# srihari-humbarwadi/retinanet-tensorflow2.x

Measured on AMD Instinct MI355X. Metric: images/sec train, ResNet50-640 RetinaNet data-parallel step (encode + fwd + loss + bwd + clip + all-reduce + SGD/EMA); inference images/s under `infer`, higher is better.
Workload: dtype bf16; 1 GPU; ResNet50-640x640 bf16 training, 32 images/GPU (BASELINE configs[2] shard: global batch 32), resnet_initial frozen, single GPU; global_batch=32, parallelism=dp1, rccl_ranks=1, comm=torch, syncbn_messages=0

## Files before the change

### include/rnet_hip.h

```cpp
#ifndef RNET_HIP_H_
#define RNET_HIP_H_

#include <stddef.h>
#include <stdint.h>

#ifdef __cplusplus
extern "C" {
#endif
#if defined(__GNUC__)
#pragma GCC visibility push(default)
#endif

typedef enum {
  RN_OK = 0,
  RN_EINVAL = -1,
  RN_ENOMEM = -2,
  RN_EHIP = -3,
  RN_ECOMM = -4,
  RN_EUNSUPPORTED = -5
} rn_status;

enum { RN_DT_F32 = 0, RN_DT_BF16 = 1 };
enum { RN_ACT_NONE = 0, RN_ACT_RELU = 1, RN_ACT_RELU6 = 2, RN_ACT_SWISH = 3 };

// ... 84 lines not shown

typedef struct {
  const void* x;
  const void* w;
  void* y;
  const float* scale;
  const float* shift;
  const void* residual;
  int32_t N, H, W, Cin, pix_stride, Ho, Wo, Cout;
  float* bn_partial;
  const float* bias;
  int32_t w_terms;
  int32_t w_pair;
  const void* bn_bwd_y;
  const float* bn_bwd_fwd;
} rn_conv_segment;

typedef struct {
  int32_t R, S, stride_h, stride_w, pad_top, pad_left;
  int32_t act;
  int32_t out_dtype;
  int32_t num_segments;
  rn_conv_segment seg[RN_CONV_MAX_SEGMENTS];
  rn_launch_opts opts;
  void* splitk_ws;
  int64_t splitk_ws_bytes;
} rn_conv_problem;

int rn_conv2d_nhwc_fwd(const rn_conv_problem* problem , void* stream);
size_t rn_conv_splitk_workspace_bytes(const rn_conv_problem* problem );
size_t rn_conv_splitk_workspace_max_bytes(void);

int rn_conv_cout_pad(int Cout);
int rn_conv_tile_rows(const rn_conv_problem* problem);
int rn_conv_bn_row_blocks(const rn_conv_problem* problem, int segment);
int rn_conv_kernel_id(const rn_conv_problem* problem);
int rn_conv_cin_pad(int Cin);
int rn_pack_conv_weight(const float* w_hwio, int R, int S, int Cin, int Cout, int Cin_pad, void* w_packed,
                        void* stream);
int rn_pack_conv_weight_split(const float* w, int layout_ohwi, int R, int S, int Cin, int Cout, int Cin_pad, int terms,
                              void* w_packed, void* stream);
int rn_conv_pair_rows(int Cout);
int rn_pack_conv_weight_pair(const float* w, int layout_ohwi, int R, int S, int Cin, int Cout, int Cin_pad,
                             void* w_packed, void* stream);
int rn_pack_conv_weight_ohwi(const float* w_ohwi, int R, int S, int Cin, int Cout, int Cin_pad, void* w_packed,
                             void* stream);
int rn_pack_stem_weight(const float* w_hwio, int Cout, void* w_packed, void* stream);
int rn_stem_padded_width(int W);
int rn_pack_stem_input(const float* images, int N, int H, int W, void* packed, void* stream);
int rn_pack_stem_weight_rs(const float* w_hwio, int R, int S, int Cout, void* w_packed, void* stream);
int rn_pack_image_nhwc4(const float* images, int N, int H, int W, int pad_top, int pad_left, int Hp, int Wp,
// ... 226 lines not shown
```

### retinanet-tensorflow2.x_amd/csrc/rn_conv.hip

```cpp
#include <map>
#include <mutex>
#include <tuple>

#include <algorithm>
#include "rn_conv_dev.h"

template <int BM, int BN, int BK, bool OUT_F32, int ABL = 0, int WM = 2, int WN = 2, int STAGES = 2, bool SPLIT = false>
__global__ void __launch_bounds__(64 * WM * WN, 2) conv_fwd_kernel(const ConvArgs args) {
  constexpr int NWAVES = WM * WN;
  constexpr int NTHREADS = 64 * NWAVES;
  constexpr int SLOTS = BK / 8;
  constexpr int RPI = 64 / SLOTS;
  constexpr int A_INSTR = BM / RPI / NWAVES;
  constexpr int B_INSTR = BN / RPI / NWAVES;
  constexpr int WTM = BM / WM, WTN = BN / WN;
  constexpr int TM = WTM / 32, TN = WTN / 32;
  constexpr int KSUB = BK / 16;
  constexpr int A_BYTES = BM * BK * 2, B_BYTES = BN * BK * 2;
  constexpr int STAGE_BYTES = A_BYTES + B_BYTES;
  static_assert(A_INSTR >= 1 && B_INSTR >= 1, "tile too small for the wave count");

  extern __shared__ __attribute__((aligned(16))) char smem[];

  int tile, part = 0;
// ... 401 lines not shown
        }
#pragma unroll
        for (int q = 0; q < 4; ++q) {
          float t = f4[q] + sbs[q];
          if (round1) t = rn_rb(t);
          if (affine) t = t * ssc[q] + ssf[q];
          if (round2) t = rn_rb(t);
          f4[q] = t;
        }
        v = make_float4(f4[0], f4[1], f4[2], f4[3]);
      } else {
        v = *(const float4*)(cl + rr * BN + ec);
      }
      const long long o = (long long)m * Cout + n;
      if (sg.residual) {
        const uint2 rv = *(const uint2*)(sg.residual + o);
        v.x += rn_bf16_to_f32((uint16_t)(rv.x & 0xffffu));
        v.y += rn_bf16_to_f32((uint16_t)(rv.x >> 16));
        v.z += rn_bf16_to_f32((uint16_t)(rv.y & 0xffffu));
        v.w += rn_bf16_to_f32((uint16_t)(rv.y >> 16));
      }
      {
        float f4[4] = {v.x, v.y, v.z, v.w};
        if (!OUT_F32 && args.act == RN_ACT_SWISH) {
#pragma unroll
          for (int q = 0; q < 4; ++q) f4[q] = rn_rb(f4[q]);
        }
        rn_apply_act_n<4>(f4, args.act);
        v = make_float4(f4[0], f4[1], f4[2], f4[3]);
      }
      if ((ABL & 8) && v.x != 123.456f) continue;
// ... 278 lines not shown
  const int mc = conv_splitk_min_chunks(p);
  if (!mc) return 0;
  long long tiles = 0;
  for (int i = 0; i < p->num_segments; ++i) {
    const rn_conv_segment& s = p->seg[i];
    tiles += rn_cdiv((long long)s.N * s.Ho * s.Wo, 256) * rn_cdiv(rn_conv_cout_pad(seg_cols(s)), 256);
  }
  long long bytes = 0;
  splitk_parts((int)tiles, mc, rn_persistent_grid(0x7fffffff, rn_num_cus(), p->opts), &bytes);
  return (size_t)bytes;
}

extern "C" int rn_conv_kernel_id(const rn_conv_problem* p) {
  if (!p || p->num_segments < 1 || p->num_segments > RN_CONV_MAX_SEGMENTS) return -1;
  return conv_pick(p);
}

extern "C" int rn_conv_bn_row_blocks(const rn_conv_problem* p, int segment) {
  if (!p || p->num_segments < 1 || p->num_segments > RN_CONV_MAX_SEGMENTS || segment < 0 || segment >= p->num_segments) return 0;
  const int kid = conv_pick(p);
  const long long M = (long long)p->seg[segment].N * p->seg[segment].Ho * p->seg[segment].Wo;
  if (kid == 1) {
    const int r = conv_big_balanced_rows(p);
    if (r) return (int)(2 * rn_cdiv(M, r));
  }
  const int rows = kid == 3 ? 512 : (kid ? 256 : 128);
  return (int)((rows / 128) * rn_cdiv(M, rows));
}

extern "C" int rn_conv_tile_rows(const rn_conv_problem* p) {
// ... 59 lines not shown
    RN_CHECK_ARG(s.Cout % 4 == 0, "rn_conv2d_nhwc_fwd: segment %d Cout=%d not a multiple of 4", i, s.Cout);
    const int cp = rn_conv_cout_pad(seg_cols(s));
    RN_CHECK_ARG((cp <= 64) == (cout_pad0 <= 64), "rn_conv2d_nhwc_fwd: segments mix Cout tile widths");
    RN_CHECK_ARG(!s.w_pair || ((big || halo512) && p->out_dtype == RN_DT_F32 && s.w_terms <= 1 && !s.scale && !s.shift &&
                               !s.residual && !s.bn_partial),
                 "rn_conv2d_nhwc_fwd: segment %d: w_pair needs an f32 launch without scale / shift / residual that the 256- / "
                 "512-row kernels take (rn_conv_kernel_id() != 0)", i);
    RN_CHECK_ARG(((uintptr_t)s.x | (uintptr_t)s.w | (uintptr_t)s.y | (uintptr_t)s.residual) % 16 == 0,
                 "rn_conv2d_nhwc_fwd: segment %d tensors must be 16-byte aligned", i);
    const long long M = (long long)s.N * s.Ho * s.Wo;
    RN_CHECK_ARG(M < (1ll << 31) && (long long)s.N * s.H * s.W * s.pix_stride * 2 < (1ll << 31),
                 "rn_conv2d_nhwc_fwd: segment %d input exceeds the 2 GiB buffer-addressing limit", i);
    ConvSegDev& d = a.seg[ii];
    d.x = (const uint16_t*)s.x; d.w = (const uint16_t*)s.w; d.y = s.y;
    d.scale = s.scale; d.shift = s.shift; d.residual = (const uint16_t*)s.residual;
    d.bn_partial = s.bn_partial;
    d.bn_y = (const uint16_t*)s.bn_bwd_y;
    d.bn_fwd = s.bn_bwd_fwd;
    if (s.bn_bwd_y) {
      RN_CHECK_ARG(s.bn_partial && s.bn_bwd_fwd && p->out_dtype == RN_DT_BF16 && !s.scale && !s.shift && !s.bias &&
                       !s.residual && p->act == RN_ACT_NONE && s.Cout % 8 == 0 && (uintptr_t)s.bn_bwd_y % 16 == 0,
                   "rn_conv2d_nhwc_fwd: segment %d: bn_bwd_y needs bn_partial + bn_bwd_fwd on a plain bf16 launch", i);
    }
    RN_CHECK_ARG((s.bn_bwd_y != nullptr) == (p->seg[0].bn_bwd_y != nullptr),
                 "rn_conv2d_nhwc_fwd: bn_bwd_y must be set on all segments or none");
    d.bias = s.bias;
    d.N = s.N; d.H = s.H; d.W = s.W; d.Cin = s.Cin; d.pix_stride = s.pix_stride;
    d.Ho = s.Ho; d.Wo = s.Wo; d.Cout = seg_cols(s);
    d.pair_cout = s.w_pair ? s.Cout : 0;
    d.rows = kid == 1 ? bal_rows : 0;
// ... 239 lines not shown
```

### retinanet-tensorflow2.x_amd/csrc/rn_conv_big.hip

```cpp
#include "rn_conv_big_epi.h"

namespace {

constexpr int BM = 256, BN = 256, BK = 32, NW = 8, STAGES = 4;
constexpr int A_BYTES = BM * BK * 2, STAGE_BYTES = (BM + BN) * BK * 2;
constexpr int RING_BYTES = STAGES * STAGE_BYTES, PATCH_BYTES = 4096;
constexpr int LDS_BYTES = RING_BYTES + NW * PATCH_BYTES;

template <bool OUT_F32, bool HAS_RES, bool BN_BWD = false>
__global__ void __launch_bounds__(512) conv_big_kernel(const ConvArgs args) {
  extern __shared__ __attribute__((aligned(16))) char smem[];
  const int total = args.total_tiles;
  const int G = gridDim.x;
  const int tid = threadIdx.x;
  const int lane = tid & 63;
  const int wave = __builtin_amdgcn_readfirstlane(tid >> 6);
  const int wave_m = wave >> 2, wave_n = wave & 3;
  const int R = args.R, S = args.S, RS = R * S;

  int i_v = blockIdx.x;
  int i_tap = 0, i_c0 = 0;
  int i_r = 0, i_s = 0;
  int g_iss = 0;
  int i_W = 0, i_PS = 0, i_Cin = 0, i_cw = 0;
  __amdgpu_buffer_rsrc_t rs_x, rs_w;
// ... 145 lines not shown
    _Pragma("unroll 1") for (int i = 1; i < args.nseg; ++i)                                           \
      if (tile__ >= args.seg[i].tile_begin) c_si = i;                                                 \
    const ConvSegDev& sg__ = args.seg[c_si];                                                          \
    const int lt__ = tile__ - sg__.tile_begin;                                                        \
    const int mt__ = rn_fdiv(lt__, sg__.n_tiles, rn_rcp((float)sg__.n_tiles));   \
    const int rows_t__ = sg__.rows ? sg__.rows : BM;                                                  \
    c_m0 = mt__ * rows_t__;                                                                           \
    c_mend = c_m0 + rows_t__ < sg__.M ? c_m0 + rows_t__ : sg__.M;                                     \
    c_chunk0 = mt__ * 2;                                                                              \
    c_n0 = (lt__ - mt__ * sg__.n_tiles) * BN;                                                         \
    c_ksteps = RS * (sg__.CinP / BK);                                                                 \
    c_k = 0;                                                                                          \
  } while (0)

  auto epilogue = [&]() __attribute__((always_inline)) {
    big_epilogue<OUT_F32, HAS_RES, BN_BWD>(acc, args, c_si, c_m0, c_n0, wave, smem + RING_BYTES + wave * PATCH_BYTES,
                                           BigEpiSrc(), c_mend, c_chunk0);
  };

  BIG_SETUP_ISSUE();
  BIG_SETUP_COMPUTE();
  big_acc_init<OUT_F32, HAS_RES>(acc, args, c_si, c_n0, wave);
#pragma unroll 1
  for (int t = 0; t < 3 && i_v < total; ++t) BIG_ISSUE_STEP();
  if (g_iss >= 3) asm volatile("s_waitcnt vmcnt(4)" ::: "memory");
  else asm volatile("s_waitcnt vmcnt(0)" ::: "memory");
  BIG_BARRIER();
  BIG_LOADSEG(0);
  if (wave_m == 1) BIG_BARRIER();

#define BIG_TILE_END()                                       \
// ... 14 lines not shown
    if (wave_m == 1) BIG_BARRIER();
    ++g;
    BIG_LOADSEG(g & 3);
    BIG_BARRIER();
  }
#undef BIG_TILE_END
#undef BIG_SETUP_COMPUTE
#undef BIG_BARRIER
#undef BIG_COMPUTESEG
#undef BIG_LOADSEG
#undef BIG_READ
#undef BIG_ISSUE_STEP
#undef BIG_SETUP_ISSUE
}

}

int rn_launch_conv_big(const ConvArgs& a, bool out_f32, const rn_launch_opts& opts, hipStream_t st) {
  static unsigned long long attr_set = 0;
  if (RN_ATTRS_NEEDED(attr_set)) {
    RN_CHECK_HIP(hipFuncSetAttribute((const void*)conv_big_kernel<false, false>,
                                     hipFuncAttributeMaxDynamicSharedMemorySize, LDS_BYTES));
    RN_CHECK_HIP(hipFuncSetAttribute((const void*)conv_big_kernel<false, true>,
                                     hipFuncAttributeMaxDynamicSharedMemorySize, LDS_BYTES));
    RN_CHECK_HIP(hipFuncSetAttribute((const void*)conv_big_kernel<true, false>,
                                     hipFuncAttributeMaxDynamicSharedMemorySize, LDS_BYTES));
    RN_CHECK_HIP(hipFuncSetAttribute((const void*)conv_big_kernel<true, true>,
                                     hipFuncAttributeMaxDynamicSharedMemorySize, LDS_BYTES));
    RN_CHECK_HIP(hipFuncSetAttribute((const void*)conv_big_kernel<false, false, true>,
                                     hipFuncAttributeMaxDynamicSharedMemorySize, LDS_BYTES));
    RN_ATTRS_DONE(attr_set);
  }
  const int grid = rn_persistent_grid(a.total_tiles, rn_num_cus(), opts);
  bool has_res = false;
  for (int i = 0; i < a.nseg; ++i) has_res = has_res || a.seg[i].residual != nullptr;
  const dim3 g3(grid), b3(512);
  if (a.seg[0].bn_y) {
    hipLaunchKernelGGL((conv_big_kernel<false, false, true>), g3, b3, LDS_BYTES, st, a);
  } else if (out_f32) {
    if (has_res) hipLaunchKernelGGL((conv_big_kernel<true, true>), g3, b3, LDS_BYTES, st, a);
    else hipLaunchKernelGGL((conv_big_kernel<true, false>), g3, b3, LDS_BYTES, st, a);
  } else {
    if (has_res) hipLaunchKernelGGL((conv_big_kernel<false, true>), g3, b3, LDS_BYTES, st, a);
    else hipLaunchKernelGGL((conv_big_kernel<false, false>), g3, b3, LDS_BYTES, st, a);
  }
  RN_CHECK_LAUNCH();
  return RN_OK;
}
```

### retinanet-tensorflow2.x_amd/csrc/rn_conv_big_epi.h

```cpp
#ifndef RN_CONV_BIG_EPI_H_
#define RN_CONV_BIG_EPI_H_
#include <type_traits>

#include "rn_conv_dev.h"

#ifdef HALO_PROF
__device__ unsigned long long g_halo_clk[48];
#define EPI_STAMP(k_) if (blockIdx.x == 0 && threadIdx.x == 0) g_halo_clk[k_] = clock64();
#else
#define EPI_STAMP(k_)
#endif

#ifdef HALO_ABLATE
#define EPI_ABLATE HALO_ABLATE
#else
#define EPI_ABLATE 0
#endif

typedef rn_h16 bf16x2_t __attribute__((ext_vector_type(2)));
typedef float f32x2_t __attribute__((ext_vector_type(2)));

__device__ __forceinline__ uint32_t pack2(float lo, float hi) {
  f32x2_t v = {lo, hi};
  bf16x2_t b = __builtin_convertvector(v, bf16x2_t);
// ... 96 lines not shown
#pragma unroll
  for (int j = 0; j < NJ; ++j)
#pragma unroll
    for (int q = 0; q < 4; ++q) {
      float a0 = __uint_as_float(v[0][j][q].x), a1 = __uint_as_float(v[0][j][q].y);
      float a2 = __uint_as_float(v[0][j][q].z), a3 = __uint_as_float(v[0][j][q].w);
#pragma unroll
      for (int p = 1; p < 4; ++p) {
        a0 += __uint_as_float(v[p][j][q].x); a1 += __uint_as_float(v[p][j][q].y);
        a2 += __uint_as_float(v[p][j][q].z); a3 += __uint_as_float(v[p][j][q].w);
      }
      t[j][q * 4] = a0; t[j][q * 4 + 1] = a1; t[j][q * 4 + 2] = a2; t[j][q * 4 + 3] = a3;
    }
}

template <bool OUT_F32, bool HAS_RES, bool BN_BWD = false, bool FROM_WS = false, int WM = 2>
__device__ __forceinline__ void big_epilogue(f32x16_t (&acc)[4][2], const ConvArgs& args, int c_si, int c_m0,
                                             int c_n0, int wave, char* patch, const BigEpiSrc src = BigEpiSrc(),
                                             int m_end = -1, int chunk0 = -1) {
  static_assert(!(BN_BWD && (OUT_F32 || HAS_RES)), "BN_BWD: plain bf16 launches only");
  constexpr bool LOADS = HAS_RES || BN_BWD;
  const int wave_m = wave / (8 / WM), wave_n = wave % (8 / WM);
  const ConvSegDev& sg = args.seg[c_si];
  const int Cout = sg.Cout, M = m_end >= 0 ? m_end : sg.M;
  const int nw0 = c_n0 + wave_n * 64;
  const int mw0 = c_m0 + wave_m * 128;
  const int elane = (int)__builtin_amdgcn_mbcnt_hi(~0u, __builtin_amdgcn_mbcnt_lo(~0u, 0u));
  const int fr = elane & 31, fh = elane >> 5;
  const int rrow = elane >> 3, ru = elane & 7;
  if (!OUT_F32) {
    const int nr = nw0 + ru * 8;
    const bool nok = nr < Cout;
    float sc[8], sf[8];
#pragma unroll
    for (int q = 0; q < 8; ++q) { sc[q] = 1.0f; sf[q] = 0.0f; }
// ... 33 lines not shown
    EPI_STAMP(12);
    const bool has_res = HAS_RES && sg.residual != nullptr;
    const uint16_t* const side = BN_BWD ? sg.bn_y : sg.residual;
    const bool has_side = BN_BWD ? true : has_res;
    const bool stats = sg.bn_partial != nullptr;
    float st0[8], st1[8];
#pragma unroll
    for (int q = 0; q < 8; ++q) st0[q] = st1[q] = 0.0f;
    char* const ybase = (char*)sg.y + ((long long)(mw0 + rrow) * Cout + nr) * 2;
    const long long row_bytes = (long long)Cout * 2;
    const int act = args.act;
    const bool clamp_lo = act == RN_ACT_RELU || act == RN_ACT_RELU6, clamp_hi = act == RN_ACT_RELU6;
    const bool affine = !BN_BWD && (sg.scale != nullptr || sg.shift != nullptr);
    const bool plain = BN_BWD || (!affine && !has_res && act != RN_ACT_SWISH);
    const bool round2 = affine && has_res;
    uint4 rv[2][LOADS ? 4 : 1];
#define BIG_RES_PREFETCH(buf_, i_)                                                                    \
_Pragma("unroll") for (int pass = 0; pass < (LOADS ? 4 : 0); ++pass) {                              \
  const int m = mw0 + (i_) * 32 + pass * 8 + rrow;                                                  \
  rv[buf_][pass] = make_uint4(0u, 0u, 0u, 0u);                                                      \
  if (has_side && nok && m < M) rv[buf_][pass] = *(const uint4*)(side + (long long)m * Cout + nr);  \
}
    const uint32_t lo2 = clamp_lo ? 0u : 0x80008000u, hi2 = clamp_hi ? RN_SIX_X2 : 0x7fff7fffu;
    auto blocks = [&](auto plain_c, auto stats_c, auto round2_c, auto swish_c) __attribute__((always_inline)) {
      constexpr bool PLAIN = decltype(plain_c)::value;
      constexpr int STATS = decltype(stats_c)::value, ROUND2 = decltype(round2_c)::value, SWISH = decltype(swish_c)::value;
      BIG_RES_PREFETCH(0, 0);
#pragma unroll
      for (int i = 0; i < 4; ++i) {
        EPI_STAMP(13 + 2 * i);
        if (i + 1 < 4) BIG_RES_PREFETCH((i + 1) & 1, i + 1);
        if (FROM_WS) big_epi_rebuild<2>(&acc[i][0], src, i, 0);
#pragma unroll
        for (int j = 0; j < 2; ++j)
#pragma unroll
          for (int g = 0; g < 4; ++g) {
            const int nl = j * 32 + g * 8 + fh * 4;
            uint2 pk;
            pk.x = pack2(acc[i][j][g * 4 + 0], acc[i][j][g * 4 + 1]);
            pk.y = pack2(acc[i][j][g * 4 + 2], acc[i][j][g * 4 + 3]);
            *(uint2*)(patch + fr * 128 + (((nl >> 3) ^ (fr & 7)) << 4) + ((((nl >> 2) ^ (fr >> 3)) & 1) << 3)) = pk;
          }
        EPI_STAMP(14 + 2 * i);
        uint4 vb[4];
#pragma unroll
        for (int pass = 0; pass < 4; ++pass) {
          const int row = pass * 8 + rrow;
          const uint4 t = *(const uint4*)(patch + row * 128 + ((ru ^ (row & 7)) << 4));
          vb[pass] = (pass & 1) ? make_uint4(t.z, t.w, t.x, t.y) : t;
        }
#pragma unroll
        for (int pass = 0; pass < 4; ++pass) {
          const int row = pass * 8 + rrow;
          const uint4 v = vb[pass];
          const int m = mw0 + i * 32 + row;
          if (m < M && nok) {
            uint4 ov;
            if (PLAIN) {
              ov.x = pk_min_i16(pk_max_i16(v.x, lo2), hi2); ov.y = pk_min_i16(pk_max_i16(v.y, lo2), hi2);
              ov.z = pk_min_i16(pk_max_i16(v.z, lo2), hi2); ov.w = pk_min_i16(pk_max_i16(v.w, lo2), hi2);
            } else {
              const uint4 r4 = HAS_RES ? rv[i & 1][LOADS ? pass : 0] : make_uint4(0u, 0u, 0u, 0u);
              float f[8] = {bf_lo(v.x), bf_hi(v.x), bf_lo(v.y), bf_hi(v.y), bf_lo(v.z), bf_hi(v.z), bf_lo(v.w), bf_hi(v.w)};
              const float rr[8] = {bf_lo(r4.x), bf_hi(r4.x), bf_lo(r4.y), bf_hi(r4.y),
                                   bf_lo(r4.z), bf_hi(r4.z), bf_lo(r4.w), bf_hi(r4.w)};
#pragma unroll
              for (int q = 0; q < 8; ++q) f[q] = f[q] * sc[q] + sf[q];
              if (ROUND2 == 1 || (ROUND2 == 2 && round2)) {
#pragma unroll
                for (int q = 0; q < 8; q += 2) {
                  const uint32_t pq = pack2(f[q], f[q + 1]);
                  f[q] = bf_lo(pq); f[q + 1] = bf_hi(pq);
                }
              }
#pragma unroll
              for (int q = 0; q < 8; ++q) f[q] += rr[q];
              if (SWISH == 1 || (SWISH == 2 && act == RN_ACT_SWISH)) {
#pragma unroll
                for (int q = 0; q < 8; ++q) f[q] = rn_swish(rn_rb(f[q]));
              }
              ov.x = pack2(f[0], f[1]); ov.y = pack2(f[2], f[3]); ov.z = pack2(f[4], f[5]); ov.w = pack2(f[6], f[7]);
              ov.x = pk_min_i16(pk_max_i16(ov.x, lo2), hi2); ov.y = pk_min_i16(pk_max_i16(ov.y, lo2), hi2);
// ... 13 lines not shown
                  st0[q] += g;
                  st1[q] += g * ((yy[q] - mu[BN_BWD ? q : 0]) * is[BN_BWD ? q : 0]);
                }
              } else {
#pragma unroll
                for (int q = 0; q < 8; ++q) { st0[q] += w[q]; st1[q] += w[q] * w[q]; }
              }
            }
          }
        }
      }
    };
    typedef std::integral_constant<int, 0> off_t;
    typedef std::integral_constant<int, 1> on_t;
    typedef std::integral_constant<int, 2> runtime_t;
    if constexpr (BN_BWD) {
      blocks(std::true_type{}, on_t{}, off_t{}, off_t{});
    } else if (plain) {
      if (stats) blocks(std::true_type{}, on_t{}, off_t{}, off_t{});
      else blocks(std::true_type{}, off_t{}, off_t{}, off_t{});
    } else if (!stats && act != RN_ACT_SWISH) {
      if (round2) blocks(std::false_type{}, off_t{}, on_t{}, off_t{});
      else blocks(std::false_type{}, off_t{}, off_t{}, off_t{});
    } else {
      blocks(std::false_type{}, runtime_t{}, runtime_t{}, runtime_t{});
    }
    EPI_STAMP(21);
    if (stats) {
#pragma unroll
      for (int q = 0; q < 8; ++q) {
#pragma unroll
// ... 67 lines not shown
```

### retinanet-tensorflow2.x_amd/csrc/rn_conv_dev.h

```cpp
#ifndef RN_CONV_DEV_H_
#define RN_CONV_DEV_H_
#include "rn_common.h"

typedef rn_h16 bf16x8_t __attribute__((ext_vector_type(8)));
typedef float f32x16_t __attribute__((ext_vector_type(16)));

#define CONV_THREADS 256

struct ConvSegDev {
  const uint16_t* x;
  const uint16_t* w;
  void* y;
  const float* scale;
  const float* shift;
  const uint16_t* residual;
  float* bn_partial;
  const float* bias;
  const uint16_t* bn_y;
  const float* bn_fwd;
  int N, H, W, Cin, pix_stride, Ho, Wo, Cout;
  int M, tile_begin, n_tiles, CinP;
  int cwrap, halo_pitch;
  int pair_cout, rows;
};


struct ConvArgs {
  int R, S, sh, sw, pt, pl, act, nseg, total_tiles, pad_;
  int split_f, split_s, vtotal, pad2_;
  float* ws;
// ... 34 lines not shown
```

### retinanet-tensorflow2.x_amd/csrc/rn_core.hip

```cpp
#include "rn_common.h"
#include <string.h>
#include <new>

static thread_local char g_rn_err[512] = "";

void rn_set_error(const char* fmt, ...) {
  va_list ap;
  va_start(ap, fmt);
  vsnprintf(g_rn_err, sizeof(g_rn_err), fmt, ap);
  va_end(ap);
}

extern "C" const char* rn_last_error(void) { return g_rn_err; }

extern "C" int rn_abi_version(void) { return 8; }

extern "C" int rn_storage_dtype(void) {
#ifdef RN_F16
  return 1;
#else
  return 0;
#endif
}

extern "C" int rn_device_ok(void) {
  int n = 0;
  if (hipGetDeviceCount(&n) != hipSuccess || n <= 0) {
    (void)hipGetLastError();
    return 0;
  }
// ... 119 lines not shown
```

### retinanet-tensorflow2.x_amd/retinanet/_C.py

```python
from __future__ import annotations

import ctypes
import logging
import os
from ctypes import (POINTER, Structure, c_char_p, c_float, c_int, c_int32, c_int64, c_longlong, c_size_t, c_uint32,
                    c_uint64, c_void_p)

_HERE = os.path.dirname(os.path.abspath(__file__))
LIB_PATH = os.environ.get("RNET_HIP_LIB") or os.path.join(_HERE, "librnet_hip.so")
LIB_PATH_F16 = os.environ.get("RNET_HIP_LIB_F16") or os.path.join(_HERE, "librnet_hip_f16.so")

RN_DT_F32, RN_DT_BF16 = 0, 1
RN_OK, RN_EINVAL, RN_ENOMEM, RN_EHIP, RN_ECOMM, RN_EUNSUPPORTED = 0, -1, -2, -3, -4, -5
RN_ACT_NONE, RN_ACT_RELU, RN_ACT_RELU6, RN_ACT_SWISH = 0, 1, 2, 3
RN_CONV_MAX_SEGMENTS = 10
ABI_VERSION = 8
PRED_W_TERMS = int(os.environ.get("RNET_PRED_W_TERMS", "2"))
ACT_IDS = {None: RN_ACT_NONE, "none": RN_ACT_NONE, "relu": RN_ACT_RELU, "relu6": RN_ACT_RELU6,
           "swish": RN_ACT_SWISH}


class RnetError(RuntimeError):
    pass


class DgradPack(Structure):
    _fields_ = [("w_ohwi", c_void_p), ("w_packed", c_void_p), ("R", c_int32), ("S", c_int32), ("Cin", c_int32),
                ("Cout", c_int32), ("Cout_pad", c_int32), ("pad_", c_int32)]


class ExampleInfo(Structure):
# ... 19 lines not shown
        for k, v in kw.items():
            setattr(o, k, int(v))
        return o


class Bottleneck64Problem(Structure):
    _fields_ = [("x", c_void_p), ("y", c_void_p), ("w_packed", c_void_p), ("affine", c_void_p), ("N", c_int32), ("H", c_int32),
                ("W", c_int32), ("Cx", c_int32), ("opts", LaunchOpts)]


class ConvSegment(Structure):
    _fields_ = [("x", c_void_p), ("w", c_void_p), ("y", c_void_p), ("scale", c_void_p), ("shift", c_void_p),
                ("residual", c_void_p), ("N", c_int32), ("H", c_int32), ("W", c_int32), ("Cin", c_int32),
                ("pix_stride", c_int32), ("Ho", c_int32), ("Wo", c_int32), ("Cout", c_int32), ("bn_partial", c_void_p),
                ("bias", c_void_p), ("w_terms", c_int32), ("w_pair", c_int32), ("bn_bwd_y", c_void_p),
                ("bn_bwd_fwd", c_void_p)]


class ConvProblem(Structure):
    _fields_ = [("R", c_int32), ("S", c_int32), ("stride_h", c_int32), ("stride_w", c_int32),
                ("pad_top", c_int32), ("pad_left", c_int32), ("act", c_int32), ("out_dtype", c_int32),
                ("num_segments", c_int32), ("seg", ConvSegment * RN_CONV_MAX_SEGMENTS), ("opts", LaunchOpts),
                ("splitk_ws", c_void_p), ("splitk_ws_bytes", c_int64)]


class WgradSegment(Structure):
    _fields_ = [("x", c_void_p), ("dy", c_void_p), ("N", c_int32), ("H", c_int32), ("W", c_int32),
                ("Cin", c_int32), ("Ho", c_int32), ("Wo", c_int32), ("Cout", c_int32),
                ("dy_pix_stride", c_int32), ("x_pix_stride", c_int32)]


# ... 57 lines not shown
                                  c_size_t, c_void_p]),
    "rn_detect_workspace_bytes": (c_size_t, [c_int, c_int64, c_int, c_int]),
    "rn_detect_per_class": (c_int, [_PP, POINTER(c_int64), c_int, c_int, c_int, c_void_p, c_int, c_float,
                                    c_float, c_float, c_int, c_void_p, c_void_p, c_void_p, c_void_p, c_void_p,
                                    c_size_t, c_void_p]),
    "rn_nms_workspace_bytes": (c_size_t, [c_int, c_int, c_int, c_int]),
    "rn_nms_per_class": (c_int, [c_void_p, c_void_p, c_int, c_int, c_int, c_float, c_float, c_float, c_int,
                                 c_void_p, c_void_p, c_void_p, c_void_p, c_void_p, c_void_p, c_size_t, c_void_p]),
    "rn_rowmax_argmax": (c_int, [c_void_p, c_int64, c_int, c_void_p, c_void_p, c_void_p]),
    "rn_conv2d_nhwc_fwd": (c_int, [POINTER(ConvProblem), c_void_p]),
    "rn_conv_cout_pad": (c_int, [c_int]),
    "rn_conv_tile_rows": (c_int, [POINTER(ConvProblem)]),
    "rn_conv_bn_row_blocks": (c_int, [POINTER(ConvProblem), c_int]),
    "rn_probe_spin": (c_int, [c_int, c_void_p]),
    "rn_conv_kernel_id": (c_int, [POINTER(ConvProblem)]),
    "rn_conv_splitk_workspace_bytes": (c_size_t, [POINTER(ConvProblem)]),
    "rn_conv_splitk_workspace_max_bytes": (c_size_t, []),
    "rn_conv_cin_pad": (c_int, [c_int]),
    "rn_depthwise_conv2d_nhwc_fwd": (c_int, [POINTER(DwProblem), c_void_p]),
    "rn_pack_depthwise_weight": (c_int, [c_void_p, c_int, c_int, c_void_p, c_void_p]),
    "rn_pack_depthwise_weight_flip": (c_int, [c_void_p, c_int, c_int, c_void_p, c_void_p]),
    "rn_depthwise_wgrad_workspace_bytes": (c_size_t, [POINTER(DwProblem)]),
    "rn_depthwise_conv2d_nhwc_wgrad": (c_int, [POINTER(DwProblem), c_void_p, c_void_p, c_size_t, c_void_p]),
    "rn_squeeze_excite_fwd": (c_int, [c_void_p, c_void_p, c_int, c_int, c_int, c_void_p, c_void_p, c_void_p, c_void_p,
                                      c_int, c_void_p, c_size_t, c_void_p]),
    "rn_squeeze_excite_bwd": (c_int, [c_void_p, c_void_p, c_void_p, c_int, c_int, c_int, c_void_p, c_void_p, c_int,
                                      c_void_p, c_void_p, c_void_p, c_void_p, c_void_p, c_void_p, c_size_t, c_void_p]),
    "rn_coco_accumulate": (c_int, [c_void_p, c_void_p, c_void_p, c_void_p, c_float, c_float, c_void_p, c_int, c_int, c_int,
                                   c_int, c_void_p, c_void_p, c_void_p]),
    "rn_pack_conv_weight_ohwi": (c_int, [c_void_p, c_int, c_int, c_int, c_int, c_int, c_void_p, c_void_p]),
# ... 299 lines not shown
```

### retinanet-tensorflow2.x_amd/retinanet/model/train_engine.py

```python
from __future__ import annotations

import ctypes
import math
import os

import numpy as np
import torch

from retinanet import _C
from .bottleneck import Bottleneck64, fused_blocks
from .forward import (FoldedConvs, conv_launch_name, conv_problem, dw_problem, half_activations, maxpool_step, split_by_depth,
                      stem_input, stem_pool_partner, stem_pool_step, stem_problem, tensor_readers, topdown_step)

_DT = {"bf16": torch.bfloat16, "f32": torch.float32}
_SEG_DTYPE = np.dtype([("offset", "<i8"), ("size", "<i8"), ("wd", "<i4"), ("bb", "<i4"), ("nb", "<i4"),
                       ("pad", "<i4"), ("bf", "<i8")])


def _hwio_to_ohwi(w):
    return w.permute(3, 0, 1, 2).contiguous()


def _ohwi_to_hwio(w):
    return w.permute(1, 2, 3, 0).contiguous()
# ... 57 lines not shown
        cus = os.environ.get("RNET_WGRAD_CUS", "160,208")
        self._wgrad_cap = tuple(int(v) for v in cus.split(",")) if cus not in ("0", "") else None
        if os.environ.get("RNET_WGRAD_STREAM", "1") == "0":
            self._wgrad_cap = None
        if self._wgrad_cap and len(self._wgrad_cap) == 1:
            self._wgrad_cap = (self._wgrad_cap[0], 2 * self._wgrad_cap[0])
        self._wgrad_capped = []
        self.step_count = 0
        self.conv_profile = None
        self.wgrad_profile = None
        self.layer_profile = None
        self.fuse_bn_stats = os.environ.get("RNET_FUSE_BN_STATS", "1") != "0"
        self.fuse_bn_bwd = os.environ.get("RNET_FUSE_BN_BWD", "1") != "0"
        self.fuse_bn_bwd_groups = os.environ.get("RNET_FUSE_BN_BWD", "1") == "2"
        self.bn_act_mask = os.environ.get("RNET_BN_ACT_MASK", "1") != "0"
        self.bn_bwd_ws = {}
        self._bn_bwd_pending = {}
        self.bn_bwd_fused = []
        self.side_stream_on = os.environ.get("RNET_WGRAD_STREAM", "1") != "0"
        self._side_stream = None
        self.drop_connect = True
        self.dc_masks = {}
        self.dc_all = self.dc_p = None
        self.dc_generator = torch.Generator(device=self.dev)
        self.dc_generator.manual_seed(1337)
        self._prepare_graph()
        with torch.cuda.device(self.dev):
            self.splitk_ws = _C.new_splitk_workspace(self.lib, self.dev)
            self.folded = FoldedConvs(self.lib, self.g, self.B, self.dev, self.h16, self.launch_opts, self.splitk_ws,
                                      self.eps, eligible=self._inference_form)
# ... 356 lines not shown
                s = p.seg[i]
                flops += 2 * s.N * s.Ho * s.Wo * p.R * p.S * s.Cin * s.Cout
                byts += 2 * s.N * s.H * s.W * s.pix_stride + osz * s.N * s.Ho * s.Wo * s.Cout + 2 * p.R * p.S * s.Cin * s.Cout
                if s.residual:
                    byts += 2 * s.N * s.Ho * s.Wo * s.Cout
        variant = None
        kid = self.lib.rn_conv_kernel_id(ctypes.byref(p))
        has_res = any(p.seg[i].residual for i in range(p.num_segments))
        bnb = bool(p.seg[0].bn_bwd_y)
        tmpl = (f"<{'true' if p.out_dtype == _C.RN_DT_F32 else 'false'}, {'true' if has_res else 'false'}, "
                f"{'true' if bnb else 'false'}>")
        if kid == 2:
            variant = "conv_halo_kernel" + tmpl[:-1] + ", false, 2> (256x256x32, 3x3 halo patch)"
        elif kid == 3:
            variant = "conv_halo_kernel" + tmpl[:-1] + ", false, 4> (512x128x32, 3x3 halo patch)"
        elif kid == 1:
            variant = "conv_big_kernel" + tmpl + " (256x256x32)"
        elif dom:
            variant = "conv_fwd_kernel<128,128,64,bf16>"
        return flops, byts, variant

    def _timed(self, launch, *sinks):
        cur = torch.cuda.current_stream(self.dev)
        e0, e1 = torch.cuda.Event(enable_timing=True), torch.cuda.Event(enable_timing=True)
        e0.record(cur)
        launch()
        e1.record(cur)
        for lst, row in sinks:
            if lst is not None:
                lst.append((e0, e1) + row)
# ... 313 lines not shown
                seen.add((op["op"], op["group"]))
                first_of_group[(op["op"], op["group"])] = i
        plan = []
        for i in range(len(ops) - 1, -1, -1):
            op = ops[i]
            if op["op"] in ("conv", "dwconv"):
                grp = op.get("group")
                if grp is None:
                    plan.append((op["op"], [op]))
                elif first_of_group[(op["op"], grp)] == i:
                    plan.append((op["op"], self._group_ops(op["op"], grp)))
            elif op["op"] in ("maxpool", "topdown", "balance", "stem", "se"):
                plan.append((op["op"], op))
        written = set()

        def mark(name):
            first = name not in written
            written.add(name)
            return first

        for kind, item in plan:
            if kind == "conv":
                self._plan_conv_backward(item, mark)
            elif kind == "dwconv":
                self._plan_dw_backward(item, mark)
            elif kind == "se":
                op = item
                x, dy, dx = self.t[op["inp"]], self.grad[op["out"]], self.grad[op["inp"]]
                mark(op["inp"])
                name, se = op["se"], self.g.ses[op["se"]]
                a = (x.data_ptr(), dy.data_ptr(), dx.data_ptr(), B, x.shape[1] * x.shape[2], se["C"],
                     self.Pbf.data_ptr() + 2 * self.bf_off[name + ":w1"],
                     self.Pbf.data_ptr() + 2 * self.bf_off[name + ":w2"], se["se"], self.se_state[op["out"]].data_ptr(),
# ... 64 lines not shown
                op = item
                names = op["tensors"]
                dout = [self.grad["bal:" + n] for n in names]
                ins = [self.t[n] for n in names]
                din = [self.grad[n] for n in names]
                for n in names:
                    mark(n)
                nsc = lib.rn_balance_features_bwd_scratch_bytes(len(names), op["mid"], B, ins[0].shape[1], ins[0].shape[2],
                                                                ins[0].shape[3])
                scratch = torch.empty((max(int(nsc), 256),), dtype=torch.uint8, device=self.dev)
                pd, pi, pn = _C.ptr_array(dout), _C.ptr_array(ins), _C.ptr_array(din)
                self._keep += [pd, pi, pn, scratch]
                a = (pd, pi, pn, self.bal_avg.data_ptr(), scratch.data_ptr(), scratch.numel(), len(names), op["mid"], B,
                     ins[0].shape[1], ins[0].shape[2], ins[0].shape[3])
                self.bwd_steps.append(lambda st, a=a: _C.check(lib.rn_balance_features_bwd(*a, st), "balance_bwd"))

    def set_wgrad_cap(self, on):
        for p, cap in self._wgrad_capped:
            p.opts.wgrad_target_blocks = cap if on else 0

    @staticmethod
    def _wgrad_bytes(p):
        b = 0
        for i in range(p.num_segments):
            s = p.seg[i]
            b += 2 * s.N * s.H * s.W * s.Cin + 2 * s.N * s.Ho * s.Wo * s.Cout
        return b + 4 * p.R * p.S * p.seg[0].Cin * p.seg[0].Cout

    def _group_wgrad_steps(self):
        lib = self.lib
# ... 89 lines not shown
        lib, B = self.lib, self.B
        if not self._conv_trainable(ops[0]) and not any(self.requires.get(o["inp"]) for o in ops):
            return
        if not self._conv_trainable(ops[0]):
            raise NotImplementedError("backward through a frozen conv that sits above trainable layers")
        live_bn = bool(self._bn_trainable(ops[0]))
        if live_bn:
            pb, sums, bsums, ws, dys, _ = self.bn_groups[ops[0]["out"]]
            for i, op in enumerate(ops):
                s = pb.seg[i]
                s.dz = self.grad[op["out"]].data_ptr()
                if op.get("residual") and self.requires.get(op["residual"]):
                    res = op["residual"]
                    s.dres = self.grad[res].data_ptr()
                    s.dres_accumulate = 0 if mark(res) else 1
            ws = self.bn_bwd_ws.get(id(pb), ws)
            self.bwd_steps.append(self._bn_bwd_step(pb, ws, bsums, ops))
            dy_of = {op["out"]: dys[i] for i, op in enumerate(ops)}
        else:
            dy_of = {}
            for op in ops:
                if op["out_dtype"] == "f32":
                    shp = list(self.t[op["out"]].shape)
                    shp[3] = (shp[3] + 63) // 64 * 64
                    dyb = torch.zeros(shp, dtype=self.h16, device=self.dev)
                    dy_of[op["out"]] = dyb
                else:
                    dyb = torch.empty_like(self.t[op["out"]])
                    dy_of[op["out"]] = dyb
                    a = (self.grad[op["out"]].data_ptr(), self.t[op["out"]].data_ptr(), dyb.data_ptr(),
# ... 238 lines not shown
                s.scale, s.shift, s.residual = None, None, None
                s.N, s.H, s.W, s.Cin, s.pix_stride = B, dy.shape[1], dy.shape[2], cw, cw
                s.Ho, s.Wo, s.Cout = dy.shape[1], dy.shape[2], c["cin"]
                continue
            if stride == 2:
                up = torch.empty((B, H, W, cw), dtype=self.h16, device=self.dev)
                ups.append((dy.data_ptr(), up.data_ptr(), B, dy.shape[1], dy.shape[2], cw, H, W))
                self._keep.append(up)
                src = up
            elif stride == 1:
                src = dy
            else:
                raise NotImplementedError("stride > 2")
            gbuf = self._gradbuf(op["inp"])
            first = mark(op["inp"] if op["inp"] not in self.bal_src else "bal:" + op["inp"])
            plain_first.append(first and stride == 1)
            s = p.seg[i]
            s.x, s.w, s.y = src.data_ptr(), packs[op["conv"]].data_ptr(), gbuf.data_ptr()
            s.scale, s.shift = None, None
            s.residual = None if first else gbuf.data_ptr()
            s.N, s.H, s.W, s.Cin, s.pix_stride = B, src.shape[1], src.shape[2], cw, cw
            s.Ho, s.Wo, s.Cout = H, W, c["cin"]
        bn_fused = 0
        hits = [self._bn_bwd_fusable(op["inp"]) for op in need] if len(plain_first) == len(need) and all(plain_first) else []
        if hits and all(h is not None for h in hits):
            for i, (op, (pb, j)) in enumerate(zip(need, hits)):
                pend = self._bn_bwd_pending.setdefault(id(pb), {"pb": pb, "seg": {}})
                if j in pend["seg"]:
                    pend["dead"] = True
                pend["seg"][j] = (p, i, op["inp"], None)
# ... 452 lines not shown
```

Measured before the change: 1121 images/s.

## Fuse ReLU-masked residual gradient join into dgrad conv epilogue

At residual joins where the BN backward writes dres and a stride-1 1x1 dgrad conv then accumulates into the same buffer, the BN backward no longer writes dres. The conv epilogue instead reads the pre-activation gradient dz and applies the ReLU activation bitmask to it on the fly. This removes one full write and one read of a bf16 activation-sized gradient tensor per join. In exchange it adds a new gated conv_big kernel variant, a cross-lane ds_bpermute of the mask words in the epilogue, and extra Python wiring that tracks which ops contribute to each gradient. The path can be turned off with RNET_RESJOIN=0.

After: 1127 images/s (median of 6 runs). No clear change (+0.6%).

```diff
diff --git a/include/rnet_hip.h b/include/rnet_hip.h
--- a/include/rnet_hip.h
+++ b/include/rnet_hip.h
@@ -122,6 +122,7 @@
   int32_t w_pair;
   const void* bn_bwd_y;
   const float* bn_bwd_fwd;
+  const void* residual_mask;
 } rn_conv_segment;
 
 typedef struct {
@@ -143,6 +144,7 @@
 int rn_conv_tile_rows(const rn_conv_problem* problem);
 int rn_conv_bn_row_blocks(const rn_conv_problem* problem, int segment);
 int rn_conv_kernel_id(const rn_conv_problem* problem);
+int rn_conv_supports_residual_mask(const rn_conv_problem* problem);
 int rn_conv_cin_pad(int Cin);
 int rn_pack_conv_weight(const float* w_hwio, int R, int S, int Cin, int Cout, int Cin_pad, void* w_packed,
                         void* stream);
diff --git a/retinanet-tensorflow2.x_amd/csrc/rn_conv.hip b/retinanet-tensorflow2.x_amd/csrc/rn_conv.hip
--- a/retinanet-tensorflow2.x_amd/csrc/rn_conv.hip
+++ b/retinanet-tensorflow2.x_amd/csrc/rn_conv.hip
@@ -439,7 +439,12 @@
       }
       const long long o = (long long)m * Cout + n;
       if (sg.residual) {
-        const uint2 rv = *(const uint2*)(sg.residual + o);
+        uint2 rv = *(const uint2*)(sg.residual + o);
+        if (sg.res_mask) {
+          const unsigned gb = (unsigned)sg.res_mask[o >> 3] >> (unsigned)(o & 4);
+          rv.x = (rv.x & ((gb & 1u) ? 0xffffu : 0u)) | (rv.x & ((gb & 2u) ? 0xffff0000u : 0u));
+          rv.y = (rv.y & ((gb & 4u) ? 0xffffu : 0u)) | (rv.y & ((gb & 8u) ? 0xffff0000u : 0u));
+        }
         v.x += rn_bf16_to_f32((uint16_t)(rv.x & 0xffffu));
         v.y += rn_bf16_to_f32((uint16_t)(rv.x >> 16));
         v.z += rn_bf16_to_f32((uint16_t)(rv.y & 0xffffu));
@@ -748,6 +753,23 @@
 extern "C" int rn_conv_kernel_id(const rn_conv_problem* p) {
   if (!p || p->num_segments < 1 || p->num_segments > RN_CONV_MAX_SEGMENTS) return -1;
   return conv_pick(p);
+}
+
+static bool conv_mask_form(const rn_conv_problem* p) {
+  if (p->out_dtype != RN_DT_BF16 || p->act != RN_ACT_NONE) return false;
+  const int kid = conv_pick(p);
+  if (kid > 1) return false;
+  const int cmul = kid == 0 ? 8 : 64;
+  for (int i = 0; i < p->num_segments; ++i) {
+    const rn_conv_segment& s = p->seg[i];
+    if (s.Cout % cmul != 0 || (uintptr_t)s.residual_mask % 4 != 0 || s.scale || s.shift || s.bias || s.bn_partial || s.bn_bwd_y || s.w_pair) return false;
+  }
+  return true;
+}
+
+extern "C" int rn_conv_supports_residual_mask(const rn_conv_problem* p) {
+  if (!p || p->num_segments < 1 || p->num_segments > RN_CONV_MAX_SEGMENTS) return 0;
+  return conv_mask_form(p) ? 1 : 0;
 }
 
 extern "C" int rn_conv_bn_row_blocks(const rn_conv_problem* p, int segment) {
@@ -837,6 +859,12 @@
     ConvSegDev& d = a.seg[ii];
     d.x = (const uint16_t*)s.x; d.w = (const uint16_t*)s.w; d.y = s.y;
     d.scale = s.scale; d.shift = s.shift; d.residual = (const uint16_t*)s.residual;
+    d.res_mask = (const unsigned char*)s.residual_mask;
+    RN_CHECK_ARG((s.residual_mask != nullptr) == (p->seg[0].residual_mask != nullptr),
+                 "rn_conv2d_nhwc_fwd: residual_mask must be set on all segments or none");
+    RN_CHECK_ARG(!s.residual_mask || (s.residual && conv_mask_form(p)),
+                 "rn_conv2d_nhwc_fwd: segment %d: residual_mask (4-byte aligned) needs a residual on a plain bf16 launch (no scale / shift / "
+                 "bias / activation / bn_partial; Cout %% 8 == 0, %% 64 on conv_big_kernel; not the halo kernel)", i);
     d.bn_partial = s.bn_partial;
     d.bn_y = (const uint16_t*)s.bn_bwd_y;
     d.bn_fwd = s.bn_bwd_fwd;
diff --git a/retinanet-tensorflow2.x_amd/csrc/rn_conv_big.hip b/retinanet-tensorflow2.x_amd/csrc/rn_conv_big.hip
--- a/retinanet-tensorflow2.x_amd/csrc/rn_conv_big.hip
+++ b/retinanet-tensorflow2.x_amd/csrc/rn_conv_big.hip
@@ -7,8 +7,8 @@
 constexpr int RING_BYTES = STAGES * STAGE_BYTES, PATCH_BYTES = 4096;
 constexpr int LDS_BYTES = RING_BYTES + NW * PATCH_BYTES;
 
-template <bool OUT_F32, bool HAS_RES, bool BN_BWD = false>
-__global__ void __launch_bounds__(512) conv_big_kernel(const ConvArgs args) {
+template <bool OUT_F32, bool HAS_RES, bool BN_BWD, bool RES_MASK>
+__device__ __forceinline__ void conv_big_body(const ConvArgs& args) {
   extern __shared__ __attribute__((aligned(16))) char smem[];
   const int total = args.total_tiles;
   const int G = gridDim.x;
@@ -184,7 +184,7 @@
   } while (0)
 
   auto epilogue = [&]() __attribute__((always_inline)) {
-    big_epilogue<OUT_F32, HAS_RES, BN_BWD>(acc, args, c_si, c_m0, c_n0, wave, smem + RING_BYTES + wave * PATCH_BYTES,
+    big_epilogue<OUT_F32, HAS_RES, BN_BWD, false, 2, RES_MASK>(acc, args, c_si, c_m0, c_n0, wave, smem + RING_BYTES + wave * PATCH_BYTES,
                                            BigEpiSrc(), c_mend, c_chunk0);
   };
 
@@ -229,6 +229,14 @@
 #undef BIG_SETUP_ISSUE
 }
 
+template <bool OUT_F32, bool HAS_RES, bool BN_BWD = false>
+__global__ void __launch_bounds__(512) conv_big_kernel(const ConvArgs args) {
+  conv_big_body<OUT_F32, HAS_RES, BN_BWD, false>(args);
+}
+__global__ void __launch_bounds__(512) conv_big_gated_kernel(const ConvArgs args) {
+  conv_big_body<false, true, false, true>(args);
+}
+
 }
 
 int rn_launch_conv_big(const ConvArgs& a, bool out_f32, const rn_launch_opts& opts, hipStream_t st) {
@@ -243,6 +251,8 @@
     RN_CHECK_HIP(hipFuncSetAttribute((const void*)conv_big_kernel<true, true>,
                                      hipFuncAttributeMaxDynamicSharedMemorySize, LDS_BYTES));
     RN_CHECK_HIP(hipFuncSetAttribute((const void*)conv_big_kernel<false, false, true>,
+                                     hipFuncAttributeMaxDynamicSharedMemorySize, LDS_BYTES));
+    RN_CHECK_HIP(hipFuncSetAttribute((const void*)conv_big_gated_kernel,
                                      hipFuncAttributeMaxDynamicSharedMemorySize, LDS_BYTES));
     RN_ATTRS_DONE(attr_set);
   }
@@ -252,6 +262,8 @@
   const dim3 g3(grid), b3(512);
   if (a.seg[0].bn_y) {
     hipLaunchKernelGGL((conv_big_kernel<false, false, true>), g3, b3, LDS_BYTES, st, a);
+  } else if (a.seg[0].res_mask) {
+    hipLaunchKernelGGL(conv_big_gated_kernel, g3, b3, LDS_BYTES, st, a);
   } else if (out_f32) {
     if (has_res) hipLaunchKernelGGL((conv_big_kernel<true, true>), g3, b3, LDS_BYTES, st, a);
     else hipLaunchKernelGGL((conv_big_kernel<true, false>), g3, b3, LDS_BYTES, st, a);
diff --git a/retinanet-tensorflow2.x_amd/csrc/rn_conv_big_epi.h b/retinanet-tensorflow2.x_amd/csrc/rn_conv_big_epi.h
--- a/retinanet-tensorflow2.x_amd/csrc/rn_conv_big_epi.h
+++ b/retinanet-tensorflow2.x_amd/csrc/rn_conv_big_epi.h
@@ -134,11 +134,12 @@
     }
 }
 
-template <bool OUT_F32, bool HAS_RES, bool BN_BWD = false, bool FROM_WS = false, int WM = 2>
+template <bool OUT_F32, bool HAS_RES, bool BN_BWD = false, bool FROM_WS = false, int WM = 2, bool RES_MASK = false>
 __device__ __forceinline__ void big_epilogue(f32x16_t (&acc)[4][2], const ConvArgs& args, int c_si, int c_m0,
                                              int c_n0, int wave, char* patch, const BigEpiSrc src = BigEpiSrc(),
                                              int m_end = -1, int chunk0 = -1) {
   static_assert(!(BN_BWD && (OUT_F32 || HAS_RES)), "BN_BWD: plain bf16 launches only");
+  static_assert(!RES_MASK || (HAS_RES && !OUT_F32), "RES_MASK: bf16 launches with a residual input only");
   constexpr bool LOADS = HAS_RES || BN_BWD;
   const int wave_m = wave / (8 / WM), wave_n = wave % (8 / WM);
   const ConvSegDev& sg = args.seg[c_si];
@@ -202,16 +203,27 @@
     const bool affine = !BN_BWD && (sg.scale != nullptr || sg.shift != nullptr);
     const bool plain = BN_BWD || (!affine && !has_res && act != RN_ACT_SWISH);
     const bool round2 = affine && has_res;
+    const unsigned char* const rmask = RES_MASK ? sg.res_mask : nullptr;
     uint4 rv[2][LOADS ? 4 : 1];
+    uint32_t rmw[2] = {0u, 0u};
+    int gsrc = (2 * rrow + (ru >> 2)) * 4, gsh = 8 * (ru & 3);
+    if (RES_MASK) asm volatile("" : "+v"(gsrc), "+v"(gsh));
 #define BIG_RES_PREFETCH(buf_, i_)                                                                    \
 _Pragma("unroll") for (int pass = 0; pass < (LOADS ? 4 : 0); ++pass) {                              \
   const int m = mw0 + (i_) * 32 + pass * 8 + rrow;                                                  \
   rv[buf_][pass] = make_uint4(0u, 0u, 0u, 0u);                                                      \
   if (has_side && nok && m < M) rv[buf_][pass] = *(const uint4*)(side + (long long)m * Cout + nr);  \
+}                                                                                                   \
+if (MASK) {                                                                                         \
+  const int m = mw0 + (i_) * 32 + (elane >> 1);                                                     \
+  rmw[buf_] = 0u;                                                                                   \
+  if (nw0 < Cout && m < M)                                                                          \
+    rmw[buf_] = *(const uint32_t*)(rmask + (((long long)m * Cout + nw0) >> 3) + 4 * (elane & 1));   \
 }
     const uint32_t lo2 = clamp_lo ? 0u : 0x80008000u, hi2 = clamp_hi ? RN_SIX_X2 : 0x7fff7fffu;
     auto blocks = [&](auto plain_c, auto stats_c, auto round2_c, auto swish_c) __attribute__((always_inline)) {
       constexpr bool PLAIN = decltype(plain_c)::value;
+      constexpr bool MASK = RES_MASK;
       constexpr int STATS = decltype(stats_c)::value, ROUND2 = decltype(round2_c)::value, SWISH = decltype(swish_c)::value;
       BIG_RES_PREFETCH(0, 0);
 #pragma unroll
@@ -236,6 +248,18 @@
           const int row = pass * 8 + rrow;
           const uint4 t = *(const uint4*)(patch + row * 128 + ((ru ^ (row & 7)) << 4));
           vb[pass] = (pass & 1) ? make_uint4(t.z, t.w, t.x, t.y) : t;
+        }
+        if (MASK) {
+#pragma unroll
+          for (int pass = 0; pass < 4; ++pass) {
+            const uint32_t w = (uint32_t)__builtin_amdgcn_ds_bpermute(gsrc + pass * 64, (int)rmw[i & 1]);
+            const uint32_t gb = w >> gsh;
+            uint4& r4 = rv[i & 1][LOADS ? pass : 0];
+#define BIG_GATE2(b_) ((bit(b_) & 0xffffu) | (bit((b_) + 1) & 0xffff0000u))
+            auto bit = [&](int b) __attribute__((always_inline)) { return (uint32_t)((int)(gb << (31 - b)) >> 31); };
+            r4.x &= BIG_GATE2(0); r4.y &= BIG_GATE2(2); r4.z &= BIG_GATE2(4); r4.w &= BIG_GATE2(6);
+#undef BIG_GATE2
+          }
         }
 #pragma unroll
         for (int pass = 0; pass < 4; ++pass) {
@@ -252,8 +276,13 @@
               float f[8] = {bf_lo(v.x), bf_hi(v.x), bf_lo(v.y), bf_hi(v.y), bf_lo(v.z), bf_hi(v.z), bf_lo(v.w), bf_hi(v.w)};
               const float rr[8] = {bf_lo(r4.x), bf_hi(r4.x), bf_lo(r4.y), bf_hi(r4.y),
                                    bf_lo(r4.z), bf_hi(r4.z), bf_lo(r4.w), bf_hi(r4.w)};
-#pragma unroll
-              for (int q = 0; q < 8; ++q) f[q] = f[q] * sc[q] + sf[q];
+              if (MASK) {
+#pragma unroll
+                for (int q = 0; q < 8; ++q) f[q] = f[q] + 0.0f;
+              } else {
+#pragma unroll
+                for (int q = 0; q < 8; ++q) f[q] = f[q] * sc[q] + sf[q];
+              }
               if (ROUND2 == 1 || (ROUND2 == 2 && round2)) {
 #pragma unroll
                 for (int q = 0; q < 8; q += 2) {
@@ -297,7 +326,9 @@
     typedef std::integral_constant<int, 0> off_t;
     typedef std::integral_constant<int, 1> on_t;
     typedef std::integral_constant<int, 2> runtime_t;
-    if constexpr (BN_BWD) {
+    if constexpr (RES_MASK) {
+      blocks(std::false_type{}, off_t{}, off_t{}, off_t{});
+    } else if constexpr (BN_BWD) {
       blocks(std::true_type{}, on_t{}, off_t{}, off_t{});
     } else if (plain) {
       if (stats) blocks(std::true_type{}, on_t{}, off_t{}, off_t{});
diff --git a/retinanet-tensorflow2.x_amd/csrc/rn_conv_dev.h b/retinanet-tensorflow2.x_amd/csrc/rn_conv_dev.h
--- a/retinanet-tensorflow2.x_amd/csrc/rn_conv_dev.h
+++ b/retinanet-tensorflow2.x_amd/csrc/rn_conv_dev.h
@@ -14,6 +14,7 @@
   const float* scale;
   const float* shift;
   const uint16_t* residual;
+  const unsigned char* res_mask;
   float* bn_partial;
   const float* bias;
   const uint16_t* bn_y;
diff --git a/retinanet-tensorflow2.x_amd/csrc/rn_core.hip b/retinanet-tensorflow2.x_amd/csrc/rn_core.hip
--- a/retinanet-tensorflow2.x_amd/csrc/rn_core.hip
+++ b/retinanet-tensorflow2.x_amd/csrc/rn_core.hip
@@ -13,7 +13,7 @@
 
 extern "C" const char* rn_last_error(void) { return g_rn_err; }
 
-extern "C" int rn_abi_version(void) { return 8; }
+extern "C" int rn_abi_version(void) { return 9; }
 
 extern "C" int rn_storage_dtype(void) {
 #ifdef RN_F16
diff --git a/retinanet-tensorflow2.x_amd/retinanet/_C.py b/retinanet-tensorflow2.x_amd/retinanet/_C.py
--- a/retinanet-tensorflow2.x_amd/retinanet/_C.py
+++ b/retinanet-tensorflow2.x_amd/retinanet/_C.py
@@ -14,7 +14,7 @@
 RN_OK, RN_EINVAL, RN_ENOMEM, RN_EHIP, RN_ECOMM, RN_EUNSUPPORTED = 0, -1, -2, -3, -4, -5
 RN_ACT_NONE, RN_ACT_RELU, RN_ACT_RELU6, RN_ACT_SWISH = 0, 1, 2, 3
 RN_CONV_MAX_SEGMENTS = 10
-ABI_VERSION = 8
+ABI_VERSION = 9
 PRED_W_TERMS = int(os.environ.get("RNET_PRED_W_TERMS", "2"))
 ACT_IDS = {None: RN_ACT_NONE, "none": RN_ACT_NONE, "relu": RN_ACT_RELU, "relu6": RN_ACT_RELU6,
            "swish": RN_ACT_SWISH}
@@ -64,7 +64,7 @@
                 ("residual", c_void_p), ("N", c_int32), ("H", c_int32), ("W", c_int32), ("Cin", c_int32),
                 ("pix_stride", c_int32), ("Ho", c_int32), ("Wo", c_int32), ("Cout", c_int32), ("bn_partial", c_void_p),
                 ("bias", c_void_p), ("w_terms", c_int32), ("w_pair", c_int32), ("bn_bwd_y", c_void_p),
-                ("bn_bwd_fwd", c_void_p)]
+                ("bn_bwd_fwd", c_void_p), ("residual_mask", c_void_p)]
 
 
 class ConvProblem(Structure):
@@ -152,6 +152,7 @@
     "rn_conv_bn_row_blocks": (c_int, [POINTER(ConvProblem), c_int]),
     "rn_probe_spin": (c_int, [c_int, c_void_p]),
     "rn_conv_kernel_id": (c_int, [POINTER(ConvProblem)]),
+    "rn_conv_supports_residual_mask": (c_int, [POINTER(ConvProblem)]),
     "rn_conv_splitk_workspace_bytes": (c_size_t, [POINTER(ConvProblem)]),
     "rn_conv_splitk_workspace_max_bytes": (c_size_t, []),
     "rn_conv_cin_pad": (c_int, [c_int]),
diff --git a/retinanet-tensorflow2.x_amd/retinanet/model/train_engine.py b/retinanet-tensorflow2.x_amd/retinanet/model/train_engine.py
--- a/retinanet-tensorflow2.x_amd/retinanet/model/train_engine.py
+++ b/retinanet-tensorflow2.x_amd/retinanet/model/train_engine.py
@@ -95,6 +95,8 @@
         self.fuse_bn_bwd = os.environ.get("RNET_FUSE_BN_BWD", "1") != "0"
         self.fuse_bn_bwd_groups = os.environ.get("RNET_FUSE_BN_BWD", "1") == "2"
         self.bn_act_mask = os.environ.get("RNET_BN_ACT_MASK", "1") != "0"
+        self.resjoin_on = os.environ.get("RNET_RESJOIN", "1") != "0"
+        self.resjoin = []
         self.bn_bwd_ws = {}
         self._bn_bwd_pending = {}
         self.bn_bwd_fused = []
@@ -481,6 +483,8 @@
             variant = "conv_halo_kernel" + tmpl[:-1] + ", false, 2> (256x256x32, 3x3 halo patch)"
         elif kid == 3:
             variant = "conv_halo_kernel" + tmpl[:-1] + ", false, 4> (512x128x32, 3x3 halo patch)"
+        elif kid == 1 and p.seg[0].residual_mask:
+            variant = "conv_big_gated_kernel (256x256x32)"
         elif kid == 1:
             variant = "conv_big_kernel" + tmpl + " (256x256x32)"
         elif dom:
@@ -824,9 +828,12 @@
                 plan.append((op["op"], op))
         written = set()
 
+        self._grad_contrib = {}
+
         def mark(name):
             first = name not in written
             written.add(name)
+            self._grad_contrib.setdefault(name, []).append(None)
             return first
 
         for kind, item in plan:
@@ -921,6 +928,30 @@
                 a = (pd, pi, pn, self.bal_avg.data_ptr(), scratch.data_ptr(), scratch.numel(), len(names), op["mid"], B,
                      ins[0].shape[1], ins[0].shape[2], ins[0].shape[3])
                 self.bwd_steps.append(lambda st, a=a: _C.check(lib.rn_balance_features_bwd(*a, st), "balance_bwd"))
+        self._wire_residual_joins()
+
+    def _wire_residual_joins(self):
+        relu = (_C.RN_ACT_RELU, _C.RN_ACT_RELU6)
+        for name, cs in self._grad_contrib.items():
+            if not self.resjoin_on or len(cs) != 2 or cs[0] is None or cs[1] is None:
+                continue
+            if cs[0][0] != "dres" or cs[1][0] != "dgrad":
+                continue
+            (_, pb, j), (_, p, i, k, stride) = cs
+            sb, sc = pb.seg[j], p.seg[i]
+            if k != 1 or stride != 1 or p.num_segments != 1 or pb.act not in relu or not sb.act_mask or not sb.dz:
+                continue
+            if sb.dres_accumulate or sb.dres != sc.y or sc.residual != sc.y:
+                continue
+            if (int(sb.P), int(sb.C)) != (sc.N * sc.Ho * sc.Wo, sc.Cout):
+                continue
+            if self.lib.rn_conv_supports_residual_mask(ctypes.byref(p)) != 1:
+                continue
+            sb.dres = None
+            sc.residual, sc.residual_mask = sb.dz, sb.act_mask
+            fl, by = self._algo[id(p)]
+            self._algo[id(p)] = (fl, by + int(sb.P) * int(sb.C) // 8)
+            self.resjoin.append(name)
 
     def set_wgrad_cap(self, on):
         for p, cap in self._wgrad_capped:
@@ -1040,6 +1071,7 @@
                     res = op["residual"]
                     s.dres = self.grad[res].data_ptr()
                     s.dres_accumulate = 0 if mark(res) else 1
+                    self._grad_contrib[res][-1] = ("dres", pb, i)
             ws = self.bn_bwd_ws.get(id(pb), ws)
             self.bwd_steps.append(self._bn_bwd_step(pb, ws, bsums, ops))
             dy_of = {op["out"]: dys[i] for i, op in enumerate(ops)}
@@ -1308,6 +1340,8 @@
                 raise NotImplementedError("stride > 2")
             gbuf = self._gradbuf(op["inp"])
             first = mark(op["inp"] if op["inp"] not in self.bal_src else "bal:" + op["inp"])
+            if op["inp"] not in self.bal_src:
+                self._grad_contrib[op["inp"]][-1] = ("dgrad", p, i, k, stride)
             plain_first.append(first and stride == 1)
             s = p.seg[i]
             s.x, s.w, s.y = src.data_ptr(), packs[op["conv"]].data_ptr(), gbuf.data_ptr()
```
